# shamim-hussain/tgt

Measured on AMD Instinct MI355X. Metric: graphs/sec training step, TGT-At 24L PCQM batch 256, 1/2/4/8 MI355X, higher is better.
Workload: dtype bf16

## Files before the change

### tgt_amd/csrc/layernorm.hip

```cpp
#include <cstdlib>
#include "common.hpp"

namespace tgt {

constexpr int kLnParts = 1536;

__device__ __forceinline__ void ln_load8(const void* p, int dtype, int64_t idx, float (&v)[8]) {
    if (dtype == TGT_F32) {
        const float4* q = reinterpret_cast<const float4*>(reinterpret_cast<const float*>(p) + idx);
        float4 a = q[0], b = q[1];
        v[0] = a.x; v[1] = a.y; v[2] = a.z; v[3] = a.w; v[4] = b.x; v[5] = b.y; v[6] = b.z; v[7] = b.w;
    } else {
        uint4 raw = ld16_stream<TGT_NT_LNLOAD != 0>(reinterpret_cast<const uint16_t*>(p) + idx);
        if (dtype == TGT_BF16) {
            bf16_t t[8];
            __builtin_memcpy(t, &raw, 16);
#pragma unroll
            for (int i = 0; i < 8; ++i) v[i] = to_f32(t[i]);
        } else {
            f16_t t[8];
            __builtin_memcpy(t, &raw, 16);
#pragma unroll
            for (int i = 0; i < 8; ++i) v[i] = to_f32(t[i]);
        }
    }
}

__device__ __forceinline__ void ln_store8(void* p, int dtype, int64_t idx, const float (&v)[8]) {
    if (dtype == TGT_F32) {
        float4* q = reinterpret_cast<float4*>(reinterpret_cast<float*>(p) + idx);
        q[0] = make_float4(v[0], v[1], v[2], v[3]);
        q[1] = make_float4(v[4], v[5], v[6], v[7]);
    } else {
        uint4 raw;
        if (dtype == TGT_BF16) {
            bf16_t t[8];
#pragma unroll
            for (int i = 0; i < 8; ++i) t[i] = from_f32<bf16_t>(v[i]);
            __builtin_memcpy(&raw, t, 16);
        } else {
            f16_t t[8];
#pragma unroll
            for (int i = 0; i < 8; ++i) t[i] = from_f32<f16_t>(v[i]);
            __builtin_memcpy(&raw, t, 16);
        }
        st16_stream<TGT_NT_LN != 0>(reinterpret_cast<uint16_t*>(p) + idx, raw);
    }
}


struct LnArgs {
    const void* x; const void* dy; void* y; void* dx;
    const float* gamma; const float* beta;
    float* mean; float* rstd; float* partial;
    int64_t rows; int C; float eps;
    int x_dtype, y_dtype, dy_dtype, dx_dtype;
    const void* res; int res_dtype; void* s_out;
    const float* scale; int64_t rows_per_sample;
    const void* ds_in; int ds_dtype; void* dx2;
    float* x_colsum;
};

template <int LPR, int VPL>
__global__ void __launch_bounds__(256) ln_fwd_kernel(const LnArgs a) {
    constexpr int RPW = 64 / LPR;
    const int lane = threadIdx.x & 63, sub = lane / LPR, gl = lane % LPR;
    const int64_t wave = (int64_t)blockIdx.x * 4 + (threadIdx.x >> 6), nwaves = (int64_t)gridDim.x * 4;
    const float invC = 1.f / a.C;
    float gam[VPL][8], bet[VPL][8];
#pragma unroll
    for (int v = 0; v < VPL; ++v) {
        const int col = (v * LPR + gl) * 8;
#pragma unroll
        for (int i = 0; i < 8; ++i) {
            gam[v][i] = col < a.C ? a.gamma[col + i] : 0.f;
            bet[v][i] = col < a.C ? a.beta[col + i] : 0.f;
        }
    }
    for (int64_t row = wave * RPW + sub; row < a.rows; row += nwaves * RPW) {
        float x[VPL][8];
        float s = 0.f;
#pragma unroll
        for (int v = 0; v < VPL; ++v) {
            const int col = (v * LPR + gl) * 8;
            if (col < a.C) {
                ln_load8(a.x, a.x_dtype, row * a.C + col, x[v]);
                if (a.res) {
                    float rr[8];
                    ln_load8(a.res, a.res_dtype, row * a.C + col, rr);
                    const float sc = a.scale ? a.scale[(uint32_t)row / (uint32_t)a.rows_per_sample] : 1.f;
#pragma unroll
                    for (int i = 0; i < 8; ++i) x[v][i] = rr[i] + x[v][i] * sc;
                    ln_store8(a.s_out, a.x_dtype, row * a.C + col, x[v]);
                    if (a.x_dtype == TGT_BF16) {
#pragma unroll
                        for (int i = 0; i < 8; ++i) x[v][i] = to_f32(from_f32<bf16_t>(x[v][i]));
                    } else if (a.x_dtype == TGT_F16) {
#pragma unroll
                        for (int i = 0; i < 8; ++i) x[v][i] = to_f32(from_f32<f16_t>(x[v][i]));
                    }
                }
            } else {
#pragma unroll
                for (int i = 0; i < 8; ++i) x[v][i] = 0.f;
            }
#pragma unroll
            for (int i = 0; i < 8; ++i) s += x[v][i];
        }
        const float mean = group_sum<LPR>(s) * invC;
        float q = 0.f;
#pragma unroll
        for (int v = 0; v < VPL; ++v) {
            const int col = (v * LPR + gl) * 8;
#pragma unroll
            for (int i = 0; i < 8; ++i) {
                const float d = col < a.C ? x[v][i] - mean : 0.f;
                q += d * d;
            }
        }
        const float rstd = rsqrtf(group_sum<LPR>(q) * invC + a.eps);
#pragma unroll
        for (int v = 0; v < VPL; ++v) {
            const int col = (v * LPR + gl) * 8;
            if (col < a.C) {
                float y[8];
#pragma unroll
                for (int i = 0; i < 8; ++i) y[i] = (x[v][i] - mean) * rstd * gam[v][i] + bet[v][i];
                ln_store8(a.y, a.y_dtype, row * a.C + col, y);
            }
        }
        if (gl == 0) {
            a.mean[row] = mean;
            a.rstd[row] = rstd;
        }
    }
}

template <int LPR, int VPL, bool CS>
__global__ void __launch_bounds__(256, VPL == 1 ? 5 : 1) ln_bwd_kernel(const LnArgs a) {
    constexpr int RPW = 64 / LPR, NP = CS ? 3 : 2;
    extern __shared__ __attribute__((aligned(16))) char smem[];
    float* red = reinterpret_cast<float*>(smem);
    const int lane = threadIdx.x & 63, sub = lane / LPR, gl = lane % LPR, w = threadIdx.x >> 6;
    const int64_t wave = (int64_t)blockIdx.x * 4 + w, nwaves = (int64_t)gridDim.x * 4;
    const float invC = 1.f / a.C;
    float gam[VPL][8], dgam[VPL][8], dbet[VPL][8], dxs[CS ? VPL : 1][8];
    constexpr bool kLdsAcc = CS && VPL == 1;
    float4* accx = reinterpret_cast<float4*>(smem) + 4 * threadIdx.x;
    if constexpr (kLdsAcc) accx[0] = accx[1] = accx[2] = accx[3] = make_float4(0.f, 0.f, 0.f, 0.f);
#pragma unroll
    for (int v = 0; v < VPL; ++v) {
        const int col = (v * LPR + gl) * 8;
#pragma unroll
        for (int i = 0; i < 8; ++i) {
            gam[v][i] = col < a.C ? a.gamma[col + i] : 0.f;
            dgam[v][i] = dbet[v][i] = 0.f;
            if constexpr (CS) dxs[v][i] = 0.f;
        }
    }
    for (int64_t row = wave * RPW + sub; row < a.rows; row += nwaves * RPW) {
        const float mean = a.mean[row], rstd = a.rstd[row];
        float xh[VPL][8], g[VPL][8];
        float s1 = 0.f, s2 = 0.f;
#pragma unroll
        for (int v = 0; v < VPL; ++v) {
            const int col = (v * LPR + gl) * 8;
            if (col < a.C) {
                float dy[8];
                ln_load8(a.x, a.x_dtype, row * a.C + col, xh[v]);
                ln_load8(a.dy, a.dy_dtype, row * a.C + col, dy);
#pragma unroll
                for (int i = 0; i < 8; ++i) {
                    xh[v][i] = (xh[v][i] - mean) * rstd;
                    g[v][i] = dy[i] * gam[v][i];
                    dgam[v][i] += dy[i] * xh[v][i];
                    if constexpr (!kLdsAcc) dbet[v][i] += dy[i];
                    s1 += g[v][i];
                    s2 += g[v][i] * xh[v][i];
                }
                if constexpr (kLdsAcc) {
                    float4 b0 = accx[2], b1 = accx[3];
                    b0.x += dy[0]; b0.y += dy[1]; b0.z += dy[2]; b0.w += dy[3];
                    b1.x += dy[4]; b1.y += dy[5]; b1.z += dy[6]; b1.w += dy[7];
                    accx[2] = b0; accx[3] = b1;
                }
            } else {
#pragma unroll
                for (int i = 0; i < 8; ++i) xh[v][i] = g[v][i] = 0.f;
            }
        }
        const float c1 = group_sum<LPR>(s1) * invC, c2 = group_sum<LPR>(s2) * invC;
#pragma unroll
        for (int v = 0; v < VPL; ++v) {
            const int col = (v * LPR + gl) * 8;
            if (col < a.C) {
                float dx[8];
#pragma unroll
                for (int i = 0; i < 8; ++i) dx[i] = rstd * (g[v][i] - c1 - xh[v][i] * c2);
                if (a.ds_in) {
                    float dd[8];
                    ln_load8(a.ds_in, a.ds_dtype, row * a.C + col, dd);
#pragma unroll
                    for (int i = 0; i < 8; ++i) dx[i] += dd[i];
                }
                ln_store8(a.dx, a.dx_dtype, row * a.C + col, dx);
                if (a.dx2 || a.scale) {
                    const float sc = a.scale ? a.scale[(uint32_t)row / (uint32_t)a.rows_per_sample] : 1.f;
#pragma unroll
                    for (int i = 0; i < 8; ++i) dx[i] *= sc;
                    if (a.dx2) ln_store8(a.dx2, a.dx_dtype, row * a.C + col, dx);
                }
                if constexpr (kLdsAcc) {
                    float4 a0 = accx[0], a1 = accx[1];
                    a0.x += dx[0]; a0.y += dx[1]; a0.z += dx[2]; a0.w += dx[3];
                    a1.x += dx[4]; a1.y += dx[5]; a1.z += dx[6]; a1.w += dx[7];
                    accx[0] = a0; accx[1] = a1;
                } else if constexpr (CS) {
#pragma unroll
                    for (int i = 0; i < 8; ++i) dxs[v][i] += dx[i];
                }
            }
        }
    }
    if constexpr (kLdsAcc) {
        const float4 a0 = accx[0], a1 = accx[1];
        dxs[0][0] = a0.x; dxs[0][1] = a0.y; dxs[0][2] = a0.z; dxs[0][3] = a0.w;
        dxs[0][4] = a1.x; dxs[0][5] = a1.y; dxs[0][6] = a1.z; dxs[0][7] = a1.w;
        const float4 b0 = accx[2], b1 = accx[3];
        dbet[0][0] = b0.x; dbet[0][1] = b0.y; dbet[0][2] = b0.z; dbet[0][3] = b0.w;
        dbet[0][4] = b1.x; dbet[0][5] = b1.y; dbet[0][6] = b1.z; dbet[0][7] = b1.w;
        __syncthreads();
    }
    constexpr int CW = VPL * LPR * 8;
#pragma unroll
    for (int v = 0; v < VPL; ++v)
#pragma unroll
        for (int i = 0; i < 8; ++i) {
            const int col = (v * LPR + gl) * 8 + i;
            red[((w * RPW + sub) * NP + 0) * CW + col] = dgam[v][i];
            red[((w * RPW + sub) * NP + 1) * CW + col] = dbet[v][i];
            if constexpr (CS) red[((w * RPW + sub) * NP + 2) * CW + col] = dxs[v][i];
        }
    __syncthreads();
    for (int idx = threadIdx.x; idx < NP * a.C; idx += 256) {
        const int which = idx / a.C, col = idx % a.C;
        float s = 0.f;
        for (int gidx = 0; gidx < 4 * RPW; ++gidx) s += red[(gidx * NP + which) * CW + col];
        a.partial[(int64_t)blockIdx.x * NP * a.C + idx] = s;
    }
}

__global__ void __launch_bounds__(256) partial_sum_kernel(const float* partial, int parts, int W, int split, float* out0,
                                                          float* out1) {
    __shared__ float red[32][9];
    const int cl = threadIdx.x & 7, sl = threadIdx.x >> 3;
    const int idx = blockIdx.x * 8 + cl;
    float s = 0.f;
    if (idx < W) {
        float s0 = 0.f, s1 = 0.f, s2 = 0.f, s3 = 0.f;
        int p = sl;
        for (; p + 96 < parts; p += 128) {
            s0 += partial[(int64_t)p * W + idx];
            s1 += partial[(int64_t)(p + 32) * W + idx];
            s2 += partial[(int64_t)(p + 64) * W + idx];
            s3 += partial[(int64_t)(p + 96) * W + idx];
        }
        for (; p < parts; p += 32) s0 += partial[(int64_t)p * W + idx];
        s = (s0 + s1) + (s2 + s3);
    }
    red[sl][cl] = s;
    __syncthreads();
    if (sl == 0 && idx < W) {
        float t = 0.f;
#pragma unroll
        for (int k = 0; k < 32; ++k) t += red[k][cl];
        if (idx < split) out0[idx] = t;
        else out1[idx - split] = t;
    }
}

template <int LPR, int VPL>
__global__ void __launch_bounds__(256) colsum_kernel(const void* x, int x_dtype, int64_t rows, int C, float* partial) {
    constexpr int RPW = 64 / LPR;
    extern __shared__ __attribute__((aligned(16))) char smem[];
    float* red = reinterpret_cast<float*>(smem);
    const int lane = threadIdx.x & 63, sub = lane / LPR, gl = lane % LPR, w = threadIdx.x >> 6;
    const int64_t wave = (int64_t)blockIdx.x * 4 + w, nwaves = (int64_t)gridDim.x * 4;
    float acc[VPL][8];
#pragma unroll
    for (int v = 0; v < VPL; ++v)
#pragma unroll
        for (int i = 0; i < 8; ++i) acc[v][i] = 0.f;
    for (int64_t row = wave * RPW + sub; row < rows; row += nwaves * RPW) {
#pragma unroll
        for (int v = 0; v < VPL; ++v) {
            const int col = (v * LPR + gl) * 8;
            if (col < C) {
                float t[8];
                ln_load8(x, x_dtype, row * C + col, t);
#pragma unroll
                for (int i = 0; i < 8; ++i) acc[v][i] += t[i];
            }
        }
    }
    constexpr int CW = VPL * LPR * 8;
#pragma unroll
    for (int v = 0; v < VPL; ++v)
#pragma unroll
        for (int i = 0; i < 8; ++i) red[(w * RPW + sub) * CW + (v * LPR + gl) * 8 + i] = acc[v][i];
    __syncthreads();
    for (int col = threadIdx.x; col < C; col += 256) {
        float s = 0.f;
        for (int g = 0; g < 4 * RPW; ++g) s += red[g * CW + col];
        partial[(int64_t)blockIdx.x * C + col] = s;
    }
}

template <int LPR, int VPL>
static int ln_launch(const LnArgs& a, bool bwd, float* dgamma, float* dbeta, hipStream_t st) {
    constexpr int RPW = 64 / LPR;
    int64_t blocks = (a.rows + 4 * RPW - 1) / (4 * RPW);
    if (!bwd) {
        constexpr int64_t cap = 4096;
        if (blocks > cap) blocks = cap;
        hipLaunchKernelGGL((ln_fwd_kernel<LPR, VPL>), dim3((unsigned)blocks), dim3(256), 0, st, a);
        return check_launch("ln_fwd_kernel");
    }
    const int parts = VPL == 1 ? 1280 : 1024;
    const bool cs = a.x_colsum != nullptr;
    const int np = cs ? 3 : 2;
    size_t lds = (size_t)4 * RPW * np * VPL * LPR * 8 * sizeof(float);
    if (cs && VPL == 1 && lds < 256 * 64) lds = 256 * 64;
    if (cs) hipLaunchKernelGGL((ln_bwd_kernel<LPR, VPL, true>), dim3(parts), dim3(256), lds, st, a);
    else hipLaunchKernelGGL((ln_bwd_kernel<LPR, VPL, false>), dim3(parts), dim3(256), lds, st, a);
    if (int e = check_launch("ln_bwd_kernel")) return e;
    hipLaunchKernelGGL(partial_sum_kernel, dim3((np * a.C + 7) / 8), dim3(256), 0, st, a.partial, parts, np * a.C, a.C,
                       dgamma, dbeta);
    return check_launch("partial_sum_kernel");
}

static int ln_dispatch(const LnArgs& a, bool bwd, float* dgamma, float* dbeta, hipStream_t st) {
    if (a.C % 8 || a.C <= 0 || a.C > 2048) return set_error(TGT_ERR_UNSUPPORTED, "layer norm: C=%d must be a multiple of 8, <= 2048", a.C);
    const int v8 = a.C / 8;
    if (v8 <= 4) return ln_launch<4, 1>(a, bwd, dgamma, dbeta, st);
    if (v8 <= 8) return ln_launch<8, 1>(a, bwd, dgamma, dbeta, st);
    if (v8 <= 16) return ln_launch<16, 1>(a, bwd, dgamma, dbeta, st);
    if (v8 <= 32) return ln_launch<32, 1>(a, bwd, dgamma, dbeta, st);
    if (v8 <= 64) return ln_launch<64, 1>(a, bwd, dgamma, dbeta, st);
    if (v8 <= 128) return ln_launch<64, 2>(a, bwd, dgamma, dbeta, st);
    return ln_launch<64, 4>(a, bwd, dgamma, dbeta, st);
}

static bool bad_dtype(int d) { return d != TGT_F32 && d != TGT_BF16 && d != TGT_F16; }

int layer_norm_fwd_run(const void* x, int x_dtype, const float* gamma, const float* beta, void* y, int y_dtype,
                       float* mean, float* rstd, int64_t rows, int C, float eps, hipStream_t st) {
    if (!x || !gamma || !beta || !y || !mean || !rstd || rows < 0) return set_error(TGT_ERR_INVALID, "layer norm fwd: null tensor");
    if (bad_dtype(x_dtype) || bad_dtype(y_dtype)) return set_error(TGT_ERR_INVALID, "layer norm fwd: bad dtype");
    if (((uintptr_t)x | (uintptr_t)y) % 16) return set_error(TGT_ERR_INVALID, "layer norm fwd: x/y must be 16-byte aligned");
    if (rows == 0) return TGT_OK;
    LnArgs a = {};
    a.x = x; a.y = y; a.gamma = gamma; a.beta = beta; a.mean = mean; a.rstd = rstd;
    a.rows = rows; a.C = C; a.eps = eps; a.x_dtype = x_dtype; a.y_dtype = y_dtype;
    return ln_dispatch(a, false, nullptr, nullptr, st);
}

int layer_norm_bwd_run(const void* dy, int dy_dtype, const void* x, int x_dtype, const float* gamma, const float* mean,
                       const float* rstd, void* dx, int dx_dtype, float* dgamma, float* dbeta, float* partial,
                       int64_t rows, int C, hipStream_t st) {
    if (!dy || !x || !gamma || !mean || !rstd || !dx || !dgamma || !dbeta || !partial || rows < 0)
        return set_error(TGT_ERR_INVALID, "layer norm bwd: null tensor");
    if (bad_dtype(x_dtype) || bad_dtype(dy_dtype) || bad_dtype(dx_dtype)) return set_error(TGT_ERR_INVALID, "layer norm bwd: bad dtype");
    if (((uintptr_t)x | (uintptr_t)dy | (uintptr_t)dx) % 16) return set_error(TGT_ERR_INVALID, "layer norm bwd: tensors must be 16-byte aligned");
    LnArgs a = {};
    a.x = x; a.dy = dy; a.dx = dx; a.gamma = gamma; a.mean = const_cast<float*>(mean); a.rstd = const_cast<float*>(rstd);
    a.partial = partial; a.rows = rows; a.C = C; a.x_dtype = x_dtype; a.dy_dtype = dy_dtype; a.dx_dtype = dx_dtype;
    return ln_dispatch(a, true, dgamma, dbeta, st);
}

int add_layer_norm_fwd_run(const void* x, int x_dtype, const void* res, int res_dtype, const float* scale,
                           int64_t rows_per_sample, void* s_out, const float* gamma, const float* beta, void* y,
                           int y_dtype, float* mean, float* rstd, int64_t rows, int C, float eps, hipStream_t st) {
    if (!x || !res || !s_out || !gamma || !beta || !y || !mean || !rstd || rows < 0)
        return set_error(TGT_ERR_INVALID, "add_layer_norm fwd: null tensor");
    if (bad_dtype(x_dtype) || bad_dtype(y_dtype) || bad_dtype(res_dtype)) return set_error(TGT_ERR_INVALID, "add_layer_norm fwd: bad dtype");
    if (scale && (rows_per_sample <= 0 || rows > 0xffffffffLL)) return set_error(TGT_ERR_INVALID, "add_layer_norm fwd: rows_per_sample (and rows < 2^32)");
    if (((uintptr_t)x | (uintptr_t)y | (uintptr_t)res | (uintptr_t)s_out) % 16) return set_error(TGT_ERR_INVALID, "add_layer_norm fwd: tensors must be 16-byte aligned");
    if (rows == 0) return TGT_OK;
    LnArgs a = {};
    a.x = x; a.y = y; a.gamma = gamma; a.beta = beta; a.mean = mean; a.rstd = rstd;
    a.rows = rows; a.C = C; a.eps = eps; a.x_dtype = x_dtype; a.y_dtype = y_dtype;
    a.res = res; a.res_dtype = res_dtype; a.s_out = s_out; a.scale = scale; a.rows_per_sample = rows_per_sample;
    return ln_dispatch(a, false, nullptr, nullptr, st);
}

int add_layer_norm_bwd_run(const void* dy, int dy_dtype, const void* s, int s_dtype, const void* ds_in, int ds_dtype,
                           const float* scale, int64_t rows_per_sample, const float* gamma, const float* mean,
                           const float* rstd, void* d_res, void* d_x, int d_dtype, float* dgamma, float* dbeta,
                           float* d_x_colsum, float* partial, int64_t rows, int C, hipStream_t st) {
    if (!dy || !s || !gamma || !mean || !rstd || !d_res || !dgamma || !dbeta || !partial || rows < 0)
        return set_error(TGT_ERR_INVALID, "add_layer_norm bwd: null tensor");
    if (bad_dtype(s_dtype) || bad_dtype(dy_dtype) || bad_dtype(d_dtype) || (ds_in && bad_dtype(ds_dtype)))
        return set_error(TGT_ERR_INVALID, "add_layer_norm bwd: bad dtype");
    if (scale && (rows_per_sample <= 0 || rows > 0xffffffffLL)) return set_error(TGT_ERR_INVALID, "add_layer_norm bwd: scale needs rows_per_sample (and rows < 2^32)");
    if (scale && !d_x && !d_x_colsum) return set_error(TGT_ERR_INVALID, "add_layer_norm bwd: scale without d_x only shapes d_x_colsum");
    if (d_x_colsum && d_x_colsum != dbeta + C)
        return set_error(TGT_ERR_INVALID, "add_layer_norm bwd: d_x_colsum must directly follow dbeta (one 2C buffer)");
    if (((uintptr_t)s | (uintptr_t)dy | (uintptr_t)d_res | (uintptr_t)d_x | (uintptr_t)ds_in) % 16)
        return set_error(TGT_ERR_INVALID, "add_layer_norm bwd: tensors must be 16-byte aligned");
    LnArgs a = {};
    a.x = s; a.dy = dy; a.dx = d_res; a.gamma = gamma; a.mean = const_cast<float*>(mean); a.rstd = const_cast<float*>(rstd);
    a.partial = partial; a.rows = rows; a.C = C; a.x_dtype = s_dtype; a.dy_dtype = dy_dtype; a.dx_dtype = d_dtype;
    a.ds_in = ds_in; a.ds_dtype = ds_dtype; a.dx2 = d_x; a.scale = scale; a.rows_per_sample = rows_per_sample;
    a.x_colsum = d_x_colsum;
    return ln_dispatch(a, true, dgamma, dbeta, st);
}

int layer_norm_parts() { return kLnParts; }

template <int LPR, int VPL>
static int colsum_launch(const void* x, int dt, int64_t rows, int C, float* out, float* partial, hipStream_t st) {
    constexpr int RPW = 64 / LPR;
    const size_t lds = (size_t)4 * RPW * VPL * LPR * 8 * sizeof(float);
    int64_t parts = (rows + 4 * RPW - 1) / (4 * RPW);
    parts = parts < 1 ? 1 : (parts > kLnParts ? kLnParts : parts);
    hipLaunchKernelGGL((colsum_kernel<LPR, VPL>), dim3((unsigned)parts), dim3(256), lds, st, x, dt, rows, C, partial);
    if (int e = check_launch("colsum_kernel")) return e;
    hipLaunchKernelGGL(partial_sum_kernel, dim3((C + 7) / 8), dim3(256), 0, st, partial, (int)parts, C, C, out, out);
    return check_launch("partial_sum_kernel");
}

int sum_rows_run(const float* x, int rows, int C, float* out, hipStream_t st) {
    if (!x || !out || rows < 0 || C <= 0) return set_error(TGT_ERR_INVALID, "sum_rows: bad arguments");
    hipLaunchKernelGGL(partial_sum_kernel, dim3((C + 7) / 8), dim3(256), 0, st, x, rows, C, C, out, out);
    return check_launch("partial_sum_kernel");
}

int colsum_run(const void* x, int x_dtype, int64_t rows, int C, float* out, float* partial, hipStream_t st) {
    if (!x || !out || !partial || rows < 0) return set_error(TGT_ERR_INVALID, "colsum: null tensor");
    if (bad_dtype(x_dtype)) return set_error(TGT_ERR_INVALID, "colsum: bad dtype");
    if (C % 8 || C <= 0 || C > 4096) return set_error(TGT_ERR_UNSUPPORTED, "colsum: C=%d must be a multiple of 8, <= 4096", C);
    if ((uintptr_t)x % 16) return set_error(TGT_ERR_INVALID, "colsum: x must be 16-byte aligned");
    const int v8 = C / 8;
    if (v8 <= 4) return colsum_launch<4, 1>(x, x_dtype, rows, C, out, partial, st);
    if (v8 <= 8) return colsum_launch<8, 1>(x, x_dtype, rows, C, out, partial, st);
    if (v8 <= 16) return colsum_launch<16, 1>(x, x_dtype, rows, C, out, partial, st);
    if (v8 <= 32) return colsum_launch<32, 1>(x, x_dtype, rows, C, out, partial, st);
    if (v8 <= 64) return colsum_launch<64, 1>(x, x_dtype, rows, C, out, partial, st);
    if (v8 <= 128) return colsum_launch<64, 2>(x, x_dtype, rows, C, out, partial, st);
    if (v8 <= 256) return colsum_launch<64, 4>(x, x_dtype, rows, C, out, partial, st);
    return colsum_launch<64, 8>(x, x_dtype, rows, C, out, partial, st);
}

}
```

### tgt_amd/knobs.py

```python
import os
from dataclasses import dataclass, fields

_SPEC = {
    'tri_split': ('TGT_TRI_SPLIT', True, 'flag', 'Q/K/V and E/G projected by two GEMMs (only without tri_proj)'),
    'tri_proj': ('TGT_TRI_PROJ', True, 'flag', 'Q/K/V projection inside the triplet forward kernel'),
    'tri_proj_infer': ('TGT_TRI_PROJ_INFER', True, 'flag', 'a projection-fused triplet forward that no backward follows does not write Q/K/V'),
    'agg_proj_infer': ('TGT_AGG_PROJ_INFER', True, 'flag', 'a triplet aggregate forward that no backward follows projects V inside the kernel (tgt_triplet_aggregate_proj_fwd)'),
    'tri_colsum': ('TGT_TRI_COLSUM', True, 'flag', 'bias gradient of the fused projection from the backward kernel'),
    'tri_skip': ('TGT_TRI_SKIP', 1, 'int', 'triplet kernels skip DropPath-dropped graphs: 0 off, 1 forward, 2 backward too'),
    'tri_ragged': ('TGT_TRI_RAGGED', False, 'flag', 'triplet attention skips the padded nodes of every graph (N <= 64): per-graph node counts from the mask, once per forward; padded positions of the edge stream then hold other finite values'),
    'tri_ragged_kb': ('TGT_TRI_RAGGED_KB', False, 'flag', 'the key-blocked triplet attention kernels (65..128 nodes) use the node counts they are given (TGT_TRI_COUNTS_KB): padded units, query tiles and key blocks are skipped; needs tri_ragged in the model'),
    'defer_sums': ('TGT_DEFER_SUMS', False, 'flag', 'closing sums of the backward collected into one launch (measured slower)'),
    'defer_max': ('TGT_DEFER_MAX', 56, 'int', 'sums per queue before it flushes itself'),
    'epi_ln_bwd': ('TGT_EPI_LN_BWD', True, 'flag', 'LayerNorm backward as the epilogue of the data-gradient GEMM'),
    'wgrad_stream': ('TGT_WGRAD_STREAM', False, 'flag', 'parameter gradients on a third stream inside the Trainer backward'),
    'wgrad_keep': ('TGT_WGRAD_KEEP', True, 'flag', 'forked operands kept referenced in a window instead of record_stream (with wgrad_stream)'),
    'wgrad_depth': ('TGT_WGRAD_DEPTH', 8, 'int', 'forks whose operands stay referenced before their origin stream waits for them'),
    'terminal_sums': ('TGT_TERMINAL_SUMS', True, 'flag', 'closing sums on the forked stream too (with wgrad_stream)'),
    'side_prio': ('TGT_SIDE_PRIO', -1, 'int', 'HIP priority of the node side stream (-1 = high)'),
    'wt_cache': ('TGT_WT_CACHE', True, 'flag', 'cached W^T for the data-gradient kernels'),
    'edge_gemm': ('TGT_EDGE_GEMM', True, 'flag', 'edge Linears on tgt_edge_linear'),
    'edge_n512': ('TGT_EDGE_N512', True, 'flag', "lin_O's and the narrow data gradients on own kernels"),
    'ffn_gelu_epi': ('TGT_FFN_GELU_EPI', True, 'flag', 'lin_W1 + GELU + dropout as one launch'),
    'ffn_gelu_bwd_epi': ('TGT_FFN_GELU_BWD_EPI', True, 'flag', 'GELU backward as the epilogue of lin_W2 data gradient'),
    'gelu_bwd_epi_colsum': ('TGT_GELU_BWD_EPI_COLSUM', True, 'flag', "lin_W1's bias gradient from the GELU_BWD epilogue"),
    'edge_k512': ('TGT_EDGE_K512', True, 'flag', 'lin_O (K = 512) + residual + LayerNorm as one launch'),
    'prescale': ('TGT_PRESCALE', True, 'flag', 'DropPath factor folded into the producer of the branch'),
    'stream_keepalive': ('TGT_STREAM_KEEPALIVE', False, 'flag', 'keep cross-stream tensors referenced instead of record_stream'),
    'node_stream': ('TGT_NODE_STREAM', True, 'flag', 'node channel on a second HIP stream'),
    'node_chain': ('TGT_NODE_CHAIN', True, 'flag', "the next layer's node projections chained on the side stream"),
    'flat_grad_dst': ('TGT_FLAT_GRAD_DST', True, 'flag', 'weight gradients written into the flat gradient buffer inside a Trainer backward'),
    'defer_edge': ('TGT_DEFER_EDGE', True, 'flag', 'closing edge residual performed by the next layer entry'),
    'own_gemm': ('TGT_OWN_GEMM', True, 'flag', 'library GEMMs of the step dispatched from cached plans (tgt_amd/gemm.py) instead of through torch: same library call, less host time'),
    'edge_wgrad': ('TGT_EDGE_WGRAD', False, 'flag', 'weight gradient of the 256 x 256 edge Linears inside their data-gradient launch (csrc/edge_wgrad.hip)'),
    'edge_wgrad_spare_cus': ('TGT_EDGE_WGRAD_SPARE_CUS', 0, 'int', 'CUs the fused data + weight gradient launch leaves to the side stream (it takes all 160 KB of LDS where it runs)'),
    'wgrad_maxp': ('TGT_WGRAD_MAXP', 128, 'int', 'cap on the row chunks of a split-M weight gradient (in-step sweep 32..256: 128)'),
    'embed_gemm': ('TGT_EMBED_GEMM', True, 'flag', "per-node mul / bias tables of the Gaussian 3-D embedding without nn.Embedding's sort-based backward (a host read)"),
    'gate_node_bwd': ('TGT_GATE_NODE_BWD', 0, 'int', "the node side stream's backward chain of a layer waits for that layer's triplet backward kernel (1) / for the projection's data-gradient GEMM behind it (2)"),
    'node_kb_bwd': ('TGT_NODE_KB_BWD', 1, 'int', 'node attention backward of 65..128 nodes on the key-blocked matrix-core kernel (0: the lane-per-head pair); the LIBRARY routes by the same variable, the host only words its slow-path notice by it'),
}
ENV_OF_LIBRARY = ('TGT_TRI_BWD2', 'TGT_TRI_BWD2_DMA', 'TGT_HIP_LIB', 'TGT_NODE_MFMA', 'TGT_NODE_MFMA16', 'TGT_NODE_KB', 'TGT_TUNING_FILE')


def _read(var, default, kind):
    raw = os.environ.get(var)
    if raw is None:
        return default
    if kind == 'int':
        return int(raw)
    return raw != '0' if default else raw == '1'


@dataclass(frozen=True)
class Knobs:
    tri_split: bool
    tri_proj: bool
    tri_proj_infer: bool
    agg_proj_infer: bool
    tri_colsum: bool
    tri_skip: int
    tri_ragged: bool
    tri_ragged_kb: bool
    defer_sums: bool
    defer_max: int
    epi_ln_bwd: bool
    wgrad_stream: bool
    wgrad_keep: bool
    wgrad_depth: int
    terminal_sums: bool
    side_prio: int
    wt_cache: bool
    edge_gemm: bool
    edge_n512: bool
    ffn_gelu_epi: bool
    ffn_gelu_bwd_epi: bool
    gelu_bwd_epi_colsum: bool
    edge_k512: bool
    prescale: bool
    stream_keepalive: bool
    node_stream: bool
    node_chain: bool
    flat_grad_dst: bool
    defer_edge: bool
    own_gemm: bool
    edge_wgrad: bool
    edge_wgrad_spare_cus: int
    wgrad_maxp: int
    embed_gemm: bool
    gate_node_bwd: int
    node_kb_bwd: int

    @classmethod
    def from_env(cls):
        return cls(**{name: _read(*_SPEC[name][:3]) for name in _SPEC})

    def non_default(self):
        out = {_SPEC[f.name][0]: getattr(self, f.name) for f in fields(self) if getattr(self, f.name) != _SPEC[f.name][1]}
        out.update({v: os.environ[v] for v in ENV_OF_LIBRARY if v in os.environ})
        return out


assert set(_SPEC) == {f.name for f in fields(Knobs)}
K = Knobs.from_env()
```

Baseline: 3255.

## Add LayerNorm and column-sum kernels sized for short tensors

Adds separate forward, backward and column-sum LayerNorm kernels for tensors with few rows (node-level tensors under a row threshold, on by default). They use a smaller grid, issue all loads before converting them, use vectorised LDS folds, and size the backward partial count to the row count, so short tensors pay less launch and reduction overhead. Node-level LayerNorms are small parts of the step and may run on the side stream, so the effect on the whole step is limited. It adds code paths and threshold constants that may not suit every shape.

```diff
diff --git a/tgt_amd/csrc/layernorm.hip b/tgt_amd/csrc/layernorm.hip
--- a/tgt_amd/csrc/layernorm.hip
+++ b/tgt_amd/csrc/layernorm.hip
@@ -316,6 +316,348 @@
     }
 }
 
+#ifndef TGT_LN_SHORT_ROWS
+#define TGT_LN_SHORT_ROWS 65536
+#endif
+#ifndef TGT_COLSUM_SHORT_ROWS
+#define TGT_COLSUM_SHORT_ROWS 16384
+#endif
+#ifndef TGT_LN_SHORT_FWD_GRID
+#define TGT_LN_SHORT_FWD_GRID 768
+#endif
+#ifndef TGT_LN_SHORT_ROWS_PER_WG
+#define TGT_LN_SHORT_ROWS_PER_WG 16
+#endif
+constexpr int64_t kLnShortRows = TGT_LN_SHORT_ROWS;
+constexpr int64_t kColsumShortRows = TGT_COLSUM_SHORT_ROWS;
+constexpr int kLnShortFwdGrid = TGT_LN_SHORT_FWD_GRID;
+constexpr int kLnShortRowsPerWg = TGT_LN_SHORT_ROWS_PER_WG;
+
+__device__ __forceinline__ void ln_issue8(const void* p, int dtype, int64_t idx, uint32_t (&r)[8]) {
+    if (dtype == TGT_F32) {
+        const uint4* q = reinterpret_cast<const uint4*>(reinterpret_cast<const float*>(p) + idx);
+        const uint4 a = q[0], b = q[1];
+        r[0] = a.x; r[1] = a.y; r[2] = a.z; r[3] = a.w; r[4] = b.x; r[5] = b.y; r[6] = b.z; r[7] = b.w;
+    } else {
+        const uint4 raw = ld16_stream<TGT_NT_LNLOAD != 0>(reinterpret_cast<const uint16_t*>(p) + idx);
+        r[0] = raw.x; r[1] = raw.y; r[2] = raw.z; r[3] = raw.w;
+        r[4] = r[5] = r[6] = r[7] = 0u;
+    }
+}
+__device__ __forceinline__ void ln_cvt8(int dtype, const uint32_t (&r)[8], float (&v)[8]) {
+    uint32_t w[8];
+#pragma unroll
+    for (int i = 0; i < 8; ++i) w[i] = r[i];
+    if (dtype == TGT_F32) {
+        asm volatile("" : "+v"(w[0]), "+v"(w[1]), "+v"(w[2]), "+v"(w[3]), "+v"(w[4]), "+v"(w[5]), "+v"(w[6]), "+v"(w[7]));
+#pragma unroll
+        for (int i = 0; i < 8; ++i) v[i] = __builtin_bit_cast(float, w[i]);
+    } else {
+        asm volatile("" : "+v"(w[0]), "+v"(w[1]), "+v"(w[2]), "+v"(w[3]));
+        if (dtype == TGT_BF16) {
+            bf16_t t[8];
+            __builtin_memcpy(t, w, 16);
+#pragma unroll
+            for (int i = 0; i < 8; ++i) v[i] = to_f32(t[i]);
+        } else {
+            f16_t t[8];
+            __builtin_memcpy(t, w, 16);
+#pragma unroll
+            for (int i = 0; i < 8; ++i) v[i] = to_f32(t[i]);
+        }
+    }
+}
+__device__ __forceinline__ void ln_param8(const float* p, int col, float (&v)[8]) {
+    if ((reinterpret_cast<uintptr_t>(p) & 15) == 0) {
+        const float4* q = reinterpret_cast<const float4*>(p + col);
+        const float4 a = q[0], b = q[1];
+        v[0] = a.x; v[1] = a.y; v[2] = a.z; v[3] = a.w; v[4] = b.x; v[5] = b.y; v[6] = b.z; v[7] = b.w;
+    } else {
+#pragma unroll
+        for (int i = 0; i < 8; ++i) v[i] = p[col + i];
+    }
+}
+
+template <int LPR, int VPL>
+__global__ void __launch_bounds__(256) ln_fwd_short_kernel(const LnArgs a) {
+    constexpr int RPW = 64 / LPR;
+    const int lane = threadIdx.x & 63, sub = lane / LPR, gl = lane % LPR;
+    const int64_t wave = (int64_t)blockIdx.x * 4 + (threadIdx.x >> 6), nwaves = (int64_t)gridDim.x * 4;
+    const float invC = 1.f / a.C;
+    int col[VPL];
+    bool on[VPL];
+    float gam[VPL][8], bet[VPL][8];
+#pragma unroll
+    for (int v = 0; v < VPL; ++v) {
+        const int c = (v * LPR + gl) * 8;
+        on[v] = c < a.C;
+        col[v] = on[v] ? c : a.C - 8;
+        ln_param8(a.gamma, col[v], gam[v]);
+        ln_param8(a.beta, col[v], bet[v]);
+    }
+    for (int64_t base = wave * RPW; base < a.rows; base += nwaves * RPW) {
+        const int64_t row = base + sub;
+        const bool live = row < a.rows;
+        const int64_t lrow = live ? row : a.rows - 1;
+        uint32_t xr[VPL][8], rr[VPL][8];
+        float x[VPL][8];
+        float sc = 1.f;
+        if (a.res) {
+            if (a.scale) sc = a.scale[(uint32_t)lrow / (uint32_t)a.rows_per_sample];
+#pragma unroll
+            for (int v = 0; v < VPL; ++v) ln_issue8(a.res, a.res_dtype, lrow * a.C + col[v], rr[v]);
+        }
+#pragma unroll
+        for (int v = 0; v < VPL; ++v) ln_issue8(a.x, a.x_dtype, lrow * a.C + col[v], xr[v]);
+#pragma unroll
+        for (int v = 0; v < VPL; ++v) {
+            ln_cvt8(a.x_dtype, xr[v], x[v]);
+            if (a.res) {
+                float r8[8];
+                ln_cvt8(a.res_dtype, rr[v], r8);
+#pragma unroll
+                for (int i = 0; i < 8; ++i) x[v][i] = r8[i] + x[v][i] * sc;
+                if (live && on[v]) ln_store8(a.s_out, a.x_dtype, row * a.C + col[v], x[v]);
+                if (a.x_dtype == TGT_BF16) {
+#pragma unroll
+                    for (int i = 0; i < 8; ++i) x[v][i] = to_f32(from_f32<bf16_t>(x[v][i]));
+                } else if (a.x_dtype == TGT_F16) {
+#pragma unroll
+                    for (int i = 0; i < 8; ++i) x[v][i] = to_f32(from_f32<f16_t>(x[v][i]));
+                }
+            }
+        }
+        float s = 0.f;
+#pragma unroll
+        for (int v = 0; v < VPL; ++v)
+#pragma unroll
+            for (int i = 0; i < 8; ++i) {
+                x[v][i] = on[v] ? x[v][i] : 0.f;
+                s += x[v][i];
+            }
+        const float mean = group_sum<LPR>(s) * invC;
+        float q = 0.f;
+#pragma unroll
+        for (int v = 0; v < VPL; ++v)
+#pragma unroll
+            for (int i = 0; i < 8; ++i) {
+                const float d = on[v] ? x[v][i] - mean : 0.f;
+                q += d * d;
+            }
+        const float rstd = rsqrtf(group_sum<LPR>(q) * invC + a.eps);
+#pragma unroll
+        for (int v = 0; v < VPL; ++v) {
+            if (live && on[v]) {
+                float y[8];
+#pragma unroll
+                for (int i = 0; i < 8; ++i) y[i] = (x[v][i] - mean) * rstd * gam[v][i] + bet[v][i];
+                ln_store8(a.y, a.y_dtype, row * a.C + col[v], y);
+            }
+        }
+        if (live && gl == 0) {
+            a.mean[row] = mean;
+            a.rstd[row] = rstd;
+        }
+    }
+}
+
+template <int LPR, int VPL>
+__device__ __forceinline__ void ln_fold_plane(float* red, const float (&acc)[VPL][8], int C, float* dst) {
+    constexpr int RPW = 64 / LPR, CW = VPL * LPR * 8;
+    const int lane = threadIdx.x & 63, sub = lane / LPR, gl = lane % LPR, w = threadIdx.x >> 6;
+#pragma unroll
+    for (int v = 0; v < VPL; ++v) {
+        float4* q = reinterpret_cast<float4*>(red + (w * RPW + sub) * CW + (v * LPR + gl) * 8);
+        q[0] = make_float4(acc[v][0], acc[v][1], acc[v][2], acc[v][3]);
+        q[1] = make_float4(acc[v][4], acc[v][5], acc[v][6], acc[v][7]);
+    }
+    __syncthreads();
+    for (int c = threadIdx.x; c < C; c += 256) {
+        float s = 0.f;
+#pragma unroll
+        for (int g = 0; g < 4 * RPW; ++g) s += red[g * CW + c];
+        dst[c] = s;
+    }
+    __syncthreads();
+}
+
+template <int LPR, int VPL, bool CS>
+__global__ void __launch_bounds__(256) ln_bwd_short_kernel(const LnArgs a) {
+    constexpr int RPW = 64 / LPR, NP = CS ? 3 : 2;
+    extern __shared__ __attribute__((aligned(16))) char smem[];
+    float* red = reinterpret_cast<float*>(smem);
+    const int lane = threadIdx.x & 63, sub = lane / LPR, gl = lane % LPR, w = threadIdx.x >> 6;
+    const int64_t wave = (int64_t)blockIdx.x * 4 + w, nwaves = (int64_t)gridDim.x * 4;
+    const float invC = 1.f / a.C;
+    int col[VPL];
+    bool on[VPL];
+    float gam[VPL][8], dgam[VPL][8], dbet[VPL][8], dxs[CS ? VPL : 1][8];
+#pragma unroll
+    for (int v = 0; v < VPL; ++v) {
+        const int c = (v * LPR + gl) * 8;
+        on[v] = c < a.C;
+        col[v] = on[v] ? c : a.C - 8;
+        ln_param8(a.gamma, col[v], gam[v]);
+#pragma unroll
+        for (int i = 0; i < 8; ++i) {
+            dgam[v][i] = dbet[v][i] = 0.f;
+            if constexpr (CS) dxs[v][i] = 0.f;
+        }
+    }
+    for (int64_t base = wave * RPW; base < a.rows; base += nwaves * RPW) {
+        const int64_t row = base + sub;
+        const bool live = row < a.rows;
+        const int64_t lrow = live ? row : a.rows - 1;
+        uint32_t xr[VPL][8], dyr[VPL][8], dsr[VPL][8];
+        const float mean = a.mean[lrow], rstd = a.rstd[lrow];
+        const float sc = a.scale ? a.scale[(uint32_t)lrow / (uint32_t)a.rows_per_sample] : 1.f;
+        if (a.ds_in) {
+#pragma unroll
+            for (int v = 0; v < VPL; ++v) ln_issue8(a.ds_in, a.ds_dtype, lrow * a.C + col[v], dsr[v]);
+        }
+#pragma unroll
+        for (int v = 0; v < VPL; ++v) ln_issue8(a.dy, a.dy_dtype, lrow * a.C + col[v], dyr[v]);
+#pragma unroll
+        for (int v = 0; v < VPL; ++v) ln_issue8(a.x, a.x_dtype, lrow * a.C + col[v], xr[v]);
+        float xh[VPL][8], g[VPL][8];
+        float s1 = 0.f, s2 = 0.f;
+#pragma unroll
+        for (int v = 0; v < VPL; ++v) {
+            const bool act = live && on[v];
+            float dy[8];
+            ln_cvt8(a.x_dtype, xr[v], xh[v]);
+            ln_cvt8(a.dy_dtype, dyr[v], dy);
+#pragma unroll
+            for (int i = 0; i < 8; ++i) {
+                xh[v][i] = act ? (xh[v][i] - mean) * rstd : 0.f;
+                dy[i] = act ? dy[i] : 0.f;
+                g[v][i] = dy[i] * gam[v][i];
+                dgam[v][i] += dy[i] * xh[v][i];
+                dbet[v][i] += dy[i];
+                s1 += g[v][i];
+                s2 += g[v][i] * xh[v][i];
+            }
+        }
+        const float c1 = group_sum<LPR>(s1) * invC, c2 = group_sum<LPR>(s2) * invC;
+#pragma unroll
+        for (int v = 0; v < VPL; ++v) {
+            if (live && on[v]) {
+                float dx[8];
+#pragma unroll
+                for (int i = 0; i < 8; ++i) dx[i] = rstd * (g[v][i] - c1 - xh[v][i] * c2);
+                if (a.ds_in) {
+                    float dd[8];
+                    ln_cvt8(a.ds_dtype, dsr[v], dd);
+#pragma unroll
+                    for (int i = 0; i < 8; ++i) dx[i] += dd[i];
+                }
+                ln_store8(a.dx, a.dx_dtype, row * a.C + col[v], dx);
+                if (a.dx2 || a.scale) {
+#pragma unroll
+                    for (int i = 0; i < 8; ++i) dx[i] *= sc;
+                    if (a.dx2) ln_store8(a.dx2, a.dx_dtype, row * a.C + col[v], dx);
+                }
+                if constexpr (CS) {
+#pragma unroll
+                    for (int i = 0; i < 8; ++i) dxs[v][i] += dx[i];
+                }
+            }
+        }
+    }
+    float* dst = a.partial + (int64_t)blockIdx.x * NP * a.C;
+    ln_fold_plane<LPR, VPL>(red, dgam, a.C, dst);
+    ln_fold_plane<LPR, VPL>(red, dbet, a.C, dst + a.C);
+    if constexpr (CS) ln_fold_plane<LPR, VPL>(red, dxs, a.C, dst + 2 * a.C);
+}
+
+template <int LPR, int VPL>
+__global__ void __launch_bounds__(256) colsum_short_kernel(const void* x, int x_dtype, int64_t rows, int C, float* partial) {
+    constexpr int RPW = 64 / LPR, U = VPL >= 4 ? 1 : (VPL >= 2 ? 2 : 4);
+    extern __shared__ __attribute__((aligned(16))) char smem[];
+    float* red = reinterpret_cast<float*>(smem);
+    const int lane = threadIdx.x & 63, sub = lane / LPR, gl = lane % LPR, w = threadIdx.x >> 6;
+    const int64_t wave = (int64_t)blockIdx.x * 4 + w, nwaves = (int64_t)gridDim.x * 4;
+    int col[VPL];
+    bool on[VPL];
+    float acc[VPL][8];
+#pragma unroll
+    for (int v = 0; v < VPL; ++v) {
+        const int c = (v * LPR + gl) * 8;
+        on[v] = c < C;
+        col[v] = on[v] ? c : C - 8;
+#pragma unroll
+        for (int i = 0; i < 8; ++i) acc[v][i] = 0.f;
+    }
+    for (int64_t base = wave * (RPW * U); base < rows; base += nwaves * (RPW * U)) {
+        uint32_t r[U][VPL][8];
+#pragma unroll
+        for (int u = 0; u < U; ++u) {
+            const int64_t row = base + u * RPW + sub;
+            const int64_t lrow = row < rows ? row : rows - 1;
+#pragma unroll
+            for (int v = 0; v < VPL; ++v) ln_issue8(x, x_dtype, lrow * C + col[v], r[u][v]);
+        }
+#pragma unroll
+        for (int u = 0; u < U; ++u) {
+            const bool live = base + u * RPW + sub < rows;
+#pragma unroll
+            for (int v = 0; v < VPL; ++v) {
+                float t[8];
+                ln_cvt8(x_dtype, r[u][v], t);
+#pragma unroll
+                for (int i = 0; i < 8; ++i) acc[v][i] += live && on[v] ? t[i] : 0.f;
+            }
+        }
+    }
+    ln_fold_plane<LPR, VPL>(red, acc, C, partial + (int64_t)blockIdx.x * C);
+}
+
+static int64_t ln_short_rows(int64_t dflt) {
+    static const long long v = [] {
+        const char* e = getenv("TGT_LN_SHORT");
+        return e ? atoll(e) : 1LL;
+    }();
+    return v <= 0 ? 0 : (v == 1 ? dflt : (int64_t)v);
+}
+
+static int short_parts(int64_t rows, int rows_per_pass) {
+    const int64_t per = rows_per_pass > kLnShortRowsPerWg ? rows_per_pass : kLnShortRowsPerWg;
+    const int64_t parts = (rows + per - 1) / per;
+    return (int)(parts < 1 ? 1 : (parts > kLnParts ? kLnParts : parts));
+}
+
+template <int LPR, int VPL>
+static int ln_short_launch(const LnArgs& a, bool bwd, float* dgamma, float* dbeta, hipStream_t st) {
+    constexpr int RPW = 64 / LPR;
+    if (!bwd) {
+        int64_t blocks = (a.rows + 4 * RPW - 1) / (4 * RPW);
+        if (blocks > kLnShortFwdGrid) blocks = kLnShortFwdGrid;
+        hipLaunchKernelGGL((ln_fwd_short_kernel<LPR, VPL>), dim3((unsigned)blocks), dim3(256), 0, st, a);
+        return check_launch("ln_fwd_short_kernel");
+    }
+    const int parts = short_parts(a.rows, 4 * RPW);
+    const bool cs = a.x_colsum != nullptr;
+    const int np = cs ? 3 : 2;
+    const size_t lds = (size_t)4 * RPW * VPL * LPR * 8 * sizeof(float);
+    if (cs) hipLaunchKernelGGL((ln_bwd_short_kernel<LPR, VPL, true>), dim3(parts), dim3(256), lds, st, a);
+    else hipLaunchKernelGGL((ln_bwd_short_kernel<LPR, VPL, false>), dim3(parts), dim3(256), lds, st, a);
+    if (int e = check_launch("ln_bwd_short_kernel")) return e;
+    hipLaunchKernelGGL(partial_sum_kernel, dim3((np * a.C + 7) / 8), dim3(256), 0, st, a.partial, parts, np * a.C, a.C,
+                       dgamma, dbeta);
+    return check_launch("partial_sum_kernel");
+}
+
+static int ln_short_dispatch(const LnArgs& a, bool bwd, float* dgamma, float* dbeta, hipStream_t st) {
+    const int v8 = a.C / 8;
+    if (v8 <= 4) return ln_short_launch<4, 1>(a, bwd, dgamma, dbeta, st);
+    if (v8 <= 8) return ln_short_launch<8, 1>(a, bwd, dgamma, dbeta, st);
+    if (v8 <= 16) return ln_short_launch<16, 1>(a, bwd, dgamma, dbeta, st);
+    if (v8 <= 32) return ln_short_launch<32, 1>(a, bwd, dgamma, dbeta, st);
+    if (v8 <= 64) return ln_short_launch<64, 1>(a, bwd, dgamma, dbeta, st);
+    if (v8 <= 96) return ln_short_launch<32, 3>(a, bwd, dgamma, dbeta, st);
+    return ln_short_launch<64, 2>(a, bwd, dgamma, dbeta, st);
+}
+
 template <int LPR, int VPL>
 static int ln_launch(const LnArgs& a, bool bwd, float* dgamma, float* dbeta, hipStream_t st) {
     constexpr int RPW = 64 / LPR;
@@ -342,6 +684,7 @@
 static int ln_dispatch(const LnArgs& a, bool bwd, float* dgamma, float* dbeta, hipStream_t st) {
     if (a.C % 8 || a.C <= 0 || a.C > 2048) return set_error(TGT_ERR_UNSUPPORTED, "layer norm: C=%d must be a multiple of 8, <= 2048", a.C);
     const int v8 = a.C / 8;
+    if (a.rows >= 1 && a.rows <= ln_short_rows(kLnShortRows) && v8 <= 128) return ln_short_dispatch(a, bwd, dgamma, dbeta, st);
     if (v8 <= 4) return ln_launch<4, 1>(a, bwd, dgamma, dbeta, st);
     if (v8 <= 8) return ln_launch<8, 1>(a, bwd, dgamma, dbeta, st);
     if (v8 <= 16) return ln_launch<16, 1>(a, bwd, dgamma, dbeta, st);
@@ -430,6 +773,17 @@
     return check_launch("partial_sum_kernel");
 }
 
+template <int LPR, int VPL>
+static int colsum_short_launch(const void* x, int dt, int64_t rows, int C, float* out, float* partial, hipStream_t st) {
+    constexpr int RPW = 64 / LPR, U = VPL >= 4 ? 1 : (VPL >= 2 ? 2 : 4);
+    const size_t lds = (size_t)4 * RPW * VPL * LPR * 8 * sizeof(float);
+    const int parts = short_parts(rows, 4 * RPW * U);
+    hipLaunchKernelGGL((colsum_short_kernel<LPR, VPL>), dim3(parts), dim3(256), lds, st, x, dt, rows, C, partial);
+    if (int e = check_launch("colsum_short_kernel")) return e;
+    hipLaunchKernelGGL(partial_sum_kernel, dim3((C + 7) / 8), dim3(256), 0, st, partial, parts, C, C, out, out);
+    return check_launch("partial_sum_kernel");
+}
+
 int sum_rows_run(const float* x, int rows, int C, float* out, hipStream_t st) {
     if (!x || !out || rows < 0 || C <= 0) return set_error(TGT_ERR_INVALID, "sum_rows: bad arguments");
     hipLaunchKernelGGL(partial_sum_kernel, dim3((C + 7) / 8), dim3(256), 0, st, x, rows, C, C, out, out);
@@ -442,6 +796,19 @@
     if (C % 8 || C <= 0 || C > 4096) return set_error(TGT_ERR_UNSUPPORTED, "colsum: C=%d must be a multiple of 8, <= 4096", C);
     if ((uintptr_t)x % 16) return set_error(TGT_ERR_INVALID, "colsum: x must be 16-byte aligned");
     const int v8 = C / 8;
+    if (rows >= 1 && rows <= ln_short_rows(kColsumShortRows)) {
+        if (v8 <= 4) return colsum_short_launch<4, 1>(x, x_dtype, rows, C, out, partial, st);
+        if (v8 <= 8) return colsum_short_launch<8, 1>(x, x_dtype, rows, C, out, partial, st);
+        if (v8 <= 16) return colsum_short_launch<16, 1>(x, x_dtype, rows, C, out, partial, st);
+        if (v8 <= 32) return colsum_short_launch<32, 1>(x, x_dtype, rows, C, out, partial, st);
+        if (v8 <= 64) return colsum_short_launch<64, 1>(x, x_dtype, rows, C, out, partial, st);
+        if (v8 <= 96) return colsum_short_launch<32, 3>(x, x_dtype, rows, C, out, partial, st);
+        if (v8 <= 128) return colsum_short_launch<64, 2>(x, x_dtype, rows, C, out, partial, st);
+        if (v8 <= 192) return colsum_short_launch<64, 3>(x, x_dtype, rows, C, out, partial, st);
+        if (v8 <= 256) return colsum_short_launch<64, 4>(x, x_dtype, rows, C, out, partial, st);
+        if (v8 <= 384) return colsum_short_launch<64, 6>(x, x_dtype, rows, C, out, partial, st);
+        return colsum_short_launch<64, 8>(x, x_dtype, rows, C, out, partial, st);
+    }
     if (v8 <= 4) return colsum_launch<4, 1>(x, x_dtype, rows, C, out, partial, st);
     if (v8 <= 8) return colsum_launch<8, 1>(x, x_dtype, rows, C, out, partial, st);
     if (v8 <= 16) return colsum_launch<16, 1>(x, x_dtype, rows, C, out, partial, st);
diff --git a/tgt_amd/knobs.py b/tgt_amd/knobs.py
--- a/tgt_amd/knobs.py
+++ b/tgt_amd/knobs.py
@@ -38,6 +38,7 @@
     'embed_gemm': ('TGT_EMBED_GEMM', True, 'flag', "per-node mul / bias tables of the Gaussian 3-D embedding without nn.Embedding's sort-based backward (a host read)"),
     'gate_node_bwd': ('TGT_GATE_NODE_BWD', 0, 'int', "the node side stream's backward chain of a layer waits for that layer's triplet backward kernel (1) / for the projection's data-gradient GEMM behind it (2)"),
     'node_kb_bwd': ('TGT_NODE_KB_BWD', 1, 'int', 'node attention backward of 65..128 nodes on the key-blocked matrix-core kernel (0: the lane-per-head pair); the LIBRARY routes by the same variable, the host only words its slow-path notice by it'),
+    'ln_short': ('TGT_LN_SHORT', 1, 'int', 'LayerNorm / column-sum kernels sized for short tensors (csrc/layernorm.hip: rows <= kLnShortRows): 0 off, 1 on, N > 1 rows <= N (threshold sweeps); read by the LIBRARY, listed here so that a benchmark line names it'),
 }
 ENV_OF_LIBRARY = ('TGT_TRI_BWD2', 'TGT_TRI_BWD2_DMA', 'TGT_HIP_LIB', 'TGT_NODE_MFMA', 'TGT_NODE_MFMA16', 'TGT_NODE_KB', 'TGT_TUNING_FILE')
 
@@ -89,6 +90,7 @@
     embed_gemm: bool
     gate_node_bwd: int
     node_kb_bwd: int
+    ln_short: int
 
     @classmethod
     def from_env(cls):
```

New measurement: 3291 (median of 6 runs). 1.1% higher.
